# vvvvvw/Sentinel

Measured on AMD Instinct MI355X. Metric: decided entries/sec (whole node) at 1M resources; % of HBM roofline, higher is better.
Workload: dtype int64/f64

## Files before the change

sentinel_amd/csrc/chain.h:

```cpp
#pragma once
#include <hip/hip_runtime.h>
#include <stdint.h>

#include "../../include/sentinel_gpu.h"
#include "dev_types.h"

namespace sg {

__device__ __forceinline__ int64_t j_d2l(double d) {
    if (d != d) return 0;
    if (d >= 9223372036854775807.0) return INT64_MAX;
    if (d <= -9223372036854775808.0) return INT64_MIN;
    return (int64_t)d;
}
__device__ __forceinline__ int32_t j_d2i(double d) {
    if (d != d) return 0;
    if (d >= 2147483647.0) return INT32_MAX;
    if (d <= -2147483648.0) return INT32_MIN;
    return (int32_t)d;
}
__device__ __forceinline__ int32_t j_iadd(int32_t a, int32_t b) { return (int32_t)((uint32_t)a + (uint32_t)b); }
__device__ __forceinline__ int64_t j_round(double a) {
    int64_t bits = __double_as_longlong(a);
    int64_t biased = (bits & 0x7ff0000000000000LL) >> 52;
// ... 89 lines not shown
__device__ __forceinline__ void bkt_add(Bkt& b, int64_t dP, int64_t dB, int64_t dS, int64_t dRT, int64_t dE, int64_t mrt) {
    b.pass += dP; b.block += dB; b.succ += dS; b.rt += dRT; b.exc += dE;
    if (mrt < b.minrt) b.minrt = mrt;
}
__device__ __forceinline__ void bkt_add_if(Bkt& b, bool c, int64_t dP, int64_t dB, int64_t dS, int64_t dRT, int64_t dE,
                                           int64_t mrt) {
    b.pass += c ? dP : 0; b.block += c ? dB : 0; b.succ += c ? dS : 0; b.rt += c ? dRT : 0; b.exc += c ? dE : 0;
    b.minrt = (c && mrt < b.minrt) ? mrt : b.minrt;
}
__device__ __forceinline__ void sec_add(Node& N, int sl, int64_t dP, int64_t dB, int64_t dS, int64_t dRT, int64_t dE,
                                        int64_t mrt) {
    bkt_add_if(N.sb[0], sl == 0, dP, dB, dS, dRT, dE, mrt);
    bkt_add_if(N.sb[1], sl == 1, dP, dB, dS, dRT, dE, mrt);
}
#define SEC_SUM(N, t, f) ((((t) - (N).sb[0].ws <= 1000 && (N).sb[0].ws >= 0) ? (N).sb[0].f : 0) + \
                          (((t) - (N).sb[1].ws <= 1000 && (N).sb[1].ws >= 0) ? (N).sb[1].f : 0))

__device__ __forceinline__ void min_flush(Node& N, Bkt* minb) {
    if (N.mslot >= 0 && (N.mst & MS_DIRTY) && !(N.mst & MS_DETACHED)) minb[N.mslot] = N.mb;
    N.mst &= ~MS_DIRTY;
}
__device__ __forceinline__ void exc_advance(Node& N, const Bkt* minb, int64_t T) {
    if (N.exc_sum_sec >= 0 && T - N.exc_sum_sec >= 60000) {
        N.exc_sum = 0;
    } else if (N.exc_sum_sec < 0) {
        int64_t s = 0;
        for (int k = 0; k < 60; ++k) {
            Bkt b = minb[k];
            if (b.ws >= T - 59000 && b.ws <= T) s += b.exc;
        }
        N.exc_sum = s;
    } else {
        const int64_t x1 = T - 60000;
        for (int64_t x = N.exc_sum_sec - 59000; x <= x1; x += 1000) {
            const int sl = (int)((x / 1000) % 60);
            const Bkt b = sl == N.pfslot ? N.pf : minb[sl];
            if (b.ws == x) N.exc_sum -= b.exc;
        }
    }
    N.exc_sum_sec = T;
}
__device__ __forceinline__ void min_current(Node& N, Bkt* minb, int64_t t, int32_t max_rt, uint32_t pflags) {
    int slot = (int)((t / 1000) % 60);
    int64_t ws = t - t % 1000;
    if (N.mslot == slot && N.mb.ws == ws) return;
    min_flush(N, minb);
    if ((pflags & PF_EXC_COUNT) && N.exc_sum_sec < ws) exc_advance(N, minb, ws);
    Bkt b = slot == N.pfslot ? N.pf : minb[slot];
    N.mslot = slot;
    N.mst = 0;
    if (N.pfslot >= -1) {
        N.pfslot = (slot + 1) % 60;
        N.pf = minb[N.pfslot];
    }
    if (b.ws == ws) { N.mb = b; return; }
    bool back = b.ws > ws;
    bkt_reset(b, ws, max_rt);
    N.mb = b;
    N.mst = back ? MS_DETACHED : MS_DIRTY;
}
__device__ __forceinline__ int64_t min_prev_pass(Node& N, Bkt* minb, int64_t t, int32_t max_rt, uint32_t pflags) {
    min_current(N, minb, t, max_rt, pflags);
    int slot = (int)(((t - 1000) / 1000) % 60);
    Bkt b = minb[slot];
    if (b.ws < 0) return 0;
    if (t - b.ws > 60000) return 0;
    if (b.ws + 1000 < t - 1000) return 0;
// ... 236 lines not shown
```

sentinel_amd/csrc/decide.hip:

```cpp
#include <hip/hip_runtime.h>
#include <stdlib.h>
#include <stdint.h>

#include "authority.h"
#include "chain.h"
#include "aux.h"
#include "pmap.h"

using namespace sg;

#define WAVE 64
#define MAXR 16
#define JMAX_FLOW 4
#define JMAX_DEG 4
#define JMAX_RL 2

__device__ __forceinline__ uint32_t lane_id() { return __lane_id(); }
__device__ __forceinline__ uint64_t lanemask_lt() {
    uint32_t l = lane_id();
    return l == 0 ? 0ull : (~0ull >> (64 - l));
}

#define J8_MAX (1u << 23)
#define SEG_ITEMS 16
// ... 1078 lines not shown
            LPROF(ktc)
        }
        if (r.kind == SG_EV_ENTRY) dec[sg.start + j] = d;
    }
    min_flush(N, C.minb);
    node_store(N, S, res, pg.pflags);
    if (L.mid != NO_ID) pm_store(S, L.mid, L.mp);
    if (L.tid != NO_ID) pm_store(S, L.tid, L.tm);
#pragma unroll
    for (int s = 0; s < NRMAX; ++s) if (s < nr) S.rstate[pg.rule_off + s] = rs[s];
#ifdef SG_KPROF
    if (kp) {
        S.dbg[32] += kta; S.dbg[33] += ktb; S.dbg[34] += ktc; S.dbg[35] += sg.len; S.dbg[36] += 1;
    }
#endif
#undef LPROF
}
template <int NRMAX>
__global__ __launch_bounds__(256) void k_lane(const SEv* __restrict__ recs, const sg_event* __restrict__ ev,
                                              const uint32_t* __restrict__ vals, const Seg* __restrict__ segs,
                                              const uint32_t* __restrict__ order, uint32_t m, DevState S, DevCfg cfg,
                                              int64_t t0, uint32_t* __restrict__ dec, uint32_t* __restrict__ bflags) {
    const uint32_t i = blockIdx.x * blockDim.x + threadIdx.x;
    if (i >= m) return;
    lane_seg<NRMAX>(recs, ev, vals, segs[order[i]], S, cfg, t0, dec, bflags, i);
}

struct MinDelta {
    int32_t p, b, s, rt, e, minrt;
};
struct LiteMin {
    int64_t T;
    MinDelta pd;
    bool fly;
    int64_t fT;
    MinDelta fd;
    Bkt fb;
};
__device__ __forceinline__ void md_zero(MinDelta& d) { d.p = d.b = d.s = d.rt = d.e = 0; d.minrt = INT32_MAX; }
__device__ __forceinline__ bool md_full(const MinDelta& d) { return (uint32_t)(d.p | d.b | d.s | d.rt | d.e) >= 0x40000000u; }
__device__ __forceinline__ Bkt md_apply(Bkt b, int64_t T, const MinDelta& d, int32_t max_rt) {
    if (b.ws > T) return b;
    if (b.ws < T) bkt_reset(b, T, max_rt);
    b.pass += d.p; b.block += d.b; b.succ += d.s; b.rt += d.rt; b.exc += d.e;
    if ((int64_t)d.minrt < b.minrt) b.minrt = d.minrt;
    return b;
}
__device__ __forceinline__ void lm_finish(LiteMin& L, Bkt* minb, int32_t max_rt) {
    if (L.fly) {
        minb[(L.fT / 1000) % 60] = md_apply(L.fb, L.fT, L.fd, max_rt);
        L.fly = false;
    }
}
__device__ __forceinline__ void lm_roll(LiteMin& L, Node& N, Bkt* minb, int64_t T, int32_t max_rt, uint32_t pflags) {
    lm_finish(L, minb, max_rt);
    if (L.T >= 0) {
        L.fb = minb[(L.T / 1000) % 60];
        L.fT = L.T;
        L.fd = L.pd;
        L.fly = true;
    }
    L.T = T;
    md_zero(L.pd);
    if ((pflags & PF_EXC_COUNT) && N.exc_sum_sec < T) {
        if (N.exc_sum_sec < 0) lm_finish(L, minb, max_rt);
        exc_advance(N, minb, T);
    }
}

#ifndef LITE_PL_WAVES
#define LITE_PL_WAVES 1
#endif
template <bool PL>
__global__ __launch_bounds__(256) __attribute__((amdgpu_waves_per_eu(PL ? LITE_PL_WAVES : 2))) void k_lite(const SEv* __restrict__ recs, const sg_event* __restrict__ ev,
                                              const uint32_t* __restrict__ vals, const Seg* __restrict__ segs,
                                              const uint32_t* __restrict__ order, uint32_t m, DevState S, DevCfg cfg,
                                              int64_t t0, uint32_t* __restrict__ dec, uint32_t* __restrict__ bflags) {
    const uint32_t i = blockIdx.x * blockDim.x + threadIdx.x;
    if (i >= m) return;
    const Seg sg = segs[order[i]];
    const uint32_t res = sg.res;
    const Prog pg = S.prog[res];
    if (((pg.xf & XF_PLITE) != 0) != PL) return;
    const int nf = pg.n_flow, nd = pg.n_degrade;
    const DRule* rules = S.rules + pg.rule_off + (PL ? 1 : 0);
    __shared__ DRule spr[PL ? 256 : 1];
    __shared__ PMap smp[PL ? 256 : 1], stm[PL ? 256 : 1];
    DRule& pr = spr[PL ? threadIdx.x : 0];
    PmLaneRef PLM{NO_ID, NO_ID, smp[PL ? threadIdx.x : 0], stm[PL ? threadIdx.x : 0]};
    if (PL) {
        pr = S.rules[pg.rule_off];
        PLM.mid = pr.pmap;
        PLM.mp = S.pmap[pr.pmap];
        PLM.tid = tmap_of(S, pg.tm_base, 0);
        if (PLM.tid != NO_ID) PLM.tm = S.pmap[PLM.tid];
    }
    double fcnt[2] = {0.0, 0.0};
    bool fthr[2] = {false, false};
    uint32_t fslot[2] = {0, 0};
    DegParam dr[2];
    uint32_t dslot[2] = {0, 0};
    RState ds[2];
#pragma unroll
    for (int k = 0; k < 2; ++k) {
        if (k < nf) {
            fcnt[k] = rules[k].count;
            fthr[k] = rules[k].grade == SG_FLOW_GRADE_THREAD;
            fslot[k] = rules[k].slot;
        }
        if (k < nd) {
            dr[k] = deg_param(rules[nf + k]);
            dslot[k] = rules[nf + k].slot;
            ds[k] = S.rstate[pg.rule_off + (PL ? 1 : 0) + nf + k];
        }
    }
#ifdef SG_KPROF
    const bool kp = S.dbg && i == 0;
    unsigned long long kt0 = kp ? __builtin_amdgcn_s_memtime() : 0, kta = 0, ktb = 0, ktc = 0, ktd = 0, ktf = 0, ktg = 0, kth = 0;
#define LPROF(acc)                                                \
    if (kp) {                                                     \
        unsigned long long _n = __builtin_amdgcn_s_memtime();     \
        acc += _n - kt0;                                          \
        kt0 = _n;                                                 \
    }
#else
#define LPROF(acc)
#endif
    Node N;
    node_load(N, S, res);
    const Ctx C{S.minb + (uint64_t)res * 60, cfg.max_rt, pg.pflags};
    LiteMin L;
    L.T = -1;
    L.fly = false;
    md_zero(L.pd);
    const bool has_chain = (N.flags & NI_CHAIN) != 0;
    const bool chain = has_chain && cfg.switch_on;
    if (sg.len && (t0 + recs[sg.start].dt) < (N.sb[0].ws > N.sb[1].ws ? N.sb[0].ws : N.sb[1].ws))
        atomicOr(bflags, BF_BACKWARD);
    uint64_t pm0 = 0, pm1 = 0, pm2 = 0, pm3 = 0;
#ifndef LITE_CH
#define LITE_CH 4
#endif
    constexpr uint32_t CH = LITE_CH;
    const uint4* r4 = reinterpret_cast<const uint4*>(recs + sg.start);
    const uint32_t qmax = sg.len ? sg.len - 1 : 0;
    uint4 cur[CH], nxt[CH];
#pragma unroll
    for (uint32_t k = 0; k < CH; ++k) cur[k] = r4[k < qmax ? k : qmax];
    LPROF(kta)
    for (uint32_t j0 = 0; j0 < sg.len; j0 += CH) {
#pragma unroll
    for (uint32_t k = 0; k < CH; ++k) nxt[k] = r4[j0 + CH + k < qmax ? j0 + CH + k : qmax];
#pragma unroll 1
    for (uint32_t k = 0; k < CH; ++k) {
        const uint4 rw = cur[0];
#pragma unroll
        for (uint32_t m = 0; m + 1 < CH; ++m) cur[m] = cur[m + 1];
        const uint32_t j = j0 + k;
        if (j >= sg.len) break;
        const int32_t rdt = (int32_t)rw.x;
        const uint32_t rx = rw.y;
        const int cntv = (int)(rw.z & 0xFFFFu);
        const int32_t rtv = (int32_t)(rw.z >> 16);
        const uint32_t kind = rw.w & 0xFFu, code = (rw.w >> 16) & 0xFFu;
        const int64_t t = t0 + rdt;
        const int64_t T = t - t % 1000;
        uint32_t d = mk_dec(ST_NOT_ENTRY, 0, 0);
        if (kind == SG_EV_ENTRY) {
            if (!chain) d = mk_dec(ST_NO_CHECK, 0, 0);
            else {
                if (T != L.T || md_full(L.pd)) lm_roll(L, N, C.minb, T, C.max_rt, C.pflags);
                uint32_t status = ST_PASS, slot = 0;
                uint64_t key = NO_KEY;
                if (PL) {
                    N.flags |= NI_PM | ni_tm(0);
                    if ((rw.w >> 8) & SG_F_HAS_ARG)
                        key = S.key_ring[(S.gbase + (vals[sg.start + j] & 0x7FFFFFFFu)) & cfg.ring_mask];
                    if (key != NO_KEY && !param_default_lane(S, pr, PLM.mp, cntv, key, t, bflags)) {
                        status = ST_BLOCK_PARAM;
                        slot = pr.slot;
                    }
                }
#pragma unroll
                for (int k = 0; k < 2; ++k) {
                    if (k < nf && status == ST_PASS) {
                        int32_t cur;
                        if (fthr[k]) cur = N.thread;
                        else { sec_current(N, t, C.max_rt); cur = j_d2i((double)SEC_SUM(N, t, pass)); }
                        if ((double)j_iadd(cur, cntv) > fcnt[k]) { status = ST_BLOCK_FLOW; slot = fslot[k]; }
                    }
                }
                LPROF(ktf)
                const int64_t exc_total = N.exc_sum;
#pragma unroll
                for (int k = 0; k < 2; ++k) {
                    if (k < nd && status == ST_PASS && !degrade_pass(N, C, dr[k], ds[k], t, &exc_total)) {
                        status = ST_BLOCK_DEGRADE;
                        slot = dslot[k];
                    }
                }
                LPROF(ktg)
                const bool passed = status == ST_PASS;
                const int sl = sec_current(N, t, C.max_rt);
                if (passed) {
                    N.thread++;
                    sec_add(N, sl, cntv, 0, 0, 0, 0, INT64_MAX);
                    L.pd.p += cntv;
                } else {
                    sec_add(N, sl, 0, cntv, 0, 0, 0, INT64_MAX);
                    L.pd.b += cntv;
                }
                LPROF(kth)
                if (PL && passed && key != NO_KEY && PLM.tid != NO_ID) thread_add_lane(S, PLM.tm, key, 1, bflags);
                d = passed ? mk_dec(ST_PASS, 0, 0) : mk_dec(status, slot, 0);
                if (passed && j < 256) {
                    const uint64_t b = 1ull << (j & 63);
                    if (j < 64) pm0 |= b; else if (j < 128) pm1 |= b; else if (j < 192) pm2 |= b; else pm3 |= b;
                }
            }
            LPROF(ktb)
        } else {
            bool eff;
            if (code == RC_NONE) eff = kind == SG_EV_EXIT ? chain : has_chain;
            else if (code == RC_PASSED) eff = true;
            else if (code == RC_NOT) eff = false;
            else {
                const uint32_t rel = rx - sg.start;
                if (rel >= j) { atomicOr(bflags, BF_BAD_REF); eff = false; }
                else if (rel < 256) {
                    const uint64_t w = rel < 64 ? pm0 : rel < 128 ? pm1 : rel < 192 ? pm2 : pm3;
                    eff = ((w >> (rel & 63)) & 1) != 0;
                } else eff = st_passed(dec[rx] & 0xFF);
            }
            if (eff && kind == SG_EV_EXIT) {
                if (T != L.T || md_full(L.pd)) lm_roll(L, N, C.minb, T, C.max_rt, C.pflags);
                const int sl = sec_current(N, t, C.max_rt);
                sec_add(N, sl, 0, 0, cntv, rtv, 0, rtv);
                L.pd.s += cntv;
                L.pd.rt += rtv;
                if (rtv < L.pd.minrt) L.pd.minrt = rtv;
                N.thread--;
                const uint32_t rfl = (rw.w >> 8) & 0xFFu;
                if (PL && (rfl & SG_F_EXIT_ARGS) && (N.flags & NI_PM) && (N.flags & ni_tm(0)) && PLM.tid != NO_ID) {
                    uint64_t ref = SG_REF_NONE;
                    if (rfl & RF_OWN_ARGS) ref = S.gbase + (vals[sg.start + j] & 0x7FFFFFFFu);
                    else if (code == RC_BATCH) ref = S.gbase + (vals[rx] & 0x7FFFFFFFu);
                    else if (code == RC_PASSED) ref = ev[vals[sg.start + j] & 0x7FFFFFFFu].aux & SG_REF_NONE;
                    if (ref != SG_REF_NONE) {
                        const uint64_t key = S.key_ring[ref & cfg.ring_mask];
                        if (key != NO_KEY) thread_add_lane(S, PLM.tm, key, -1, bflags);
                    }
                }
            } else if (eff && cntv > 0) {
                if (T != L.T || md_full(L.pd)) lm_roll(L, N, C.minb, T, C.max_rt, C.pflags);
                const int sl = sec_current(N, t, C.max_rt);
                sec_add(N, sl, 0, 0, 0, 0, cntv, INT64_MAX);
                L.pd.e += cntv;
                if (N.exc_sum_sec == T) N.exc_sum += cntv;
            }
            LPROF(ktc)
        }
        if (kind == SG_EV_ENTRY) dec[sg.start + j] = d;
    }
#pragma unroll
    for (uint32_t k = 0; k < CH; ++k) cur[k] = nxt[k];
    }
    lm_finish(L, C.minb, C.max_rt);
    if (L.T >= 0) {
        Bkt* b = C.minb + (L.T / 1000) % 60;
        *b = md_apply(*b, L.T, L.pd, C.max_rt);
    }
    node_store(N, S, res, pg.pflags);
#pragma unroll
    for (int k = 0; k < 2; ++k)
        if (k < nd) S.rstate[pg.rule_off + (PL ? 1 : 0) + nf + k] = ds[k];
    if (PL) {
        pm_store(S, PLM.mid, PLM.mp);
        if (PLM.tid != NO_ID) pm_store(S, PLM.tid, PLM.tm);
    }
    LPROF(ktd)
#ifdef SG_KPROF
    if (kp) {
        S.dbg[32] += kta; S.dbg[33] += ktb; S.dbg[34] += ktc; S.dbg[35] += sg.len; S.dbg[36] += 1; S.dbg[37] += ktd; S.dbg[38] += ktf; S.dbg[39] += ktg; S.dbg[51] += kth;
    }
#endif
#undef LPROF
}

#define DPP_STEP(v, ident, ctrl, rmask, OP) \
    v = OP((uint32_t)__builtin_amdgcn_update_dpp((int)(ident), (int)(v), ctrl, rmask, 0xf, false), v)
#define WAVE_SCAN(v, ident, OP)              \
    do {                                      \
        DPP_STEP(v, ident, 0x111, 0xf, OP);   \
        DPP_STEP(v, ident, 0x112, 0xf, OP);   \
        DPP_STEP(v, ident, 0x114, 0xf, OP);   \
        DPP_STEP(v, ident, 0x118, 0xf, OP);   \
        DPP_STEP(v, ident, 0x142, 0xa, OP);   \
        DPP_STEP(v, ident, 0x143, 0xc, OP);   \
    } while (0)
__device__ __forceinline__ uint32_t op_add(uint32_t a, uint32_t b) { return a + b; }
__device__ __forceinline__ uint32_t op_min(uint32_t a, uint32_t b) { return a < b ? a : b; }
__device__ __forceinline__ uint32_t op_max(uint32_t a, uint32_t b) { return a > b ? a : b; }
__device__ __forceinline__ void wave_total64(uint32_t v, uint64_t* dst) {
    uint32_t lo = v & 0xFFFFu, hi = v >> 16;
// ... 2346 lines not shown
```

sentinel_amd/csrc/dev_types.h:

```cpp
#pragma once
#include <hip/hip_runtime.h>
#include <stdint.h>

#include "../../include/sentinel_gpu.h"

namespace sg {

struct AuthDesc;

struct Bkt {
    int64_t ws;
    int64_t pass;
    int64_t block;
    int64_t exc;
    int64_t succ;
    int64_t rt;
    int64_t occ;
    int64_t minrt;
};
static_assert(sizeof(Bkt) == 64, "Bkt must be 64 B");

#define NO_KEY 0xFFFFFFFFFFFFFFFFull

enum : uint32_t {
// ... 114 lines not shown
    int64_t stamp[PM_BKT];
};
static_assert(sizeof(PBucket) == 128, "PBucket must be one 128-byte line");
struct PData {
    int64_t v0;
    int32_t v1;
    uint32_t pad;
};
static_assert(sizeof(PData) == 16, "PData must be 16 B");
#define PM_MIN_NB 2u
enum { PC_NEXT = 0, PC_FLOOR = 1, PC_RESCUES = 2, PC_RESCUE = 3, PC_WORDS = 4 };
__host__ __device__ inline uint32_t map_buckets(uint32_t cap) { return (2u * cap + PM_BKT - 1) / PM_BKT > 2u ? (2u * cap + PM_BKT - 1) / PM_BKT : 2u; }
struct PMap {
    uint64_t base;
    uint64_t bm;
    int64_t clock;
    int64_t thr;
    uint32_t nb;
    uint32_t cap;
    uint32_t live;
    uint32_t rb_log2;
    uint32_t pad[4];
};
static_assert(sizeof(PMap) == 64, "PMap must be 64 B");
#define PM_BASE_CAP 4000u
#define PM_TOTAL_CAP 200000u
#define PQ_MAX_CAP 8176u

enum : uint8_t { ST_PASS = 0, ST_PASS_WAIT = 1, ST_BLOCK_FLOW = 2, ST_BLOCK_DEGRADE = 3, ST_BLOCK_PARAM = 4,
                 ST_NO_CHECK = 5, ST_BLOCK_UPSTREAM = 6, ST_BLOCK_AUTHORITY = 7, ST_NOT_ENTRY = 0xFF };

#define HEAD_OFF 16384u
#define TABLES_ALL 32768u
struct DevCfg {
    int32_t max_rt;
    int32_t occupy_timeout;
    int32_t max_chain;
    int32_t switch_on;
    uint64_t reserved0;
    uint64_t ring_mask;
    uint32_t dbg_flags;
    uint32_t heads;
};

struct Seg {
    uint32_t res;
    uint32_t start;
    uint32_t len;
    uint32_t bin;
};
#define SEG_AUXP 0x80u
#define SEG_PV 0x40u
#define SEG_PVT 0x100u

struct PvSeg {
    uint32_t ok;
    uint32_t n;
    uint32_t off;
    uint32_t mid;
    uint32_t rk;
    uint32_t ch0;
    uint32_t nch;
    uint32_t fbits;
    uint32_t freach;
    int32_t peak;
    uint32_t tm0;
    uint32_t sub;
};

struct PvBuf {
    uint64_t* key;
    uint32_t* pos;
// ... 135 lines not shown
    unsigned long long* dbg;
    uint32_t* sink;
    const Link* link;
    const uint32_t* bst;
    uint32_t* pend;
    Span* spans;
    uint32_t* nspan;
    uint32_t span_cap;
    uint32_t epoch;
    uint32_t skip_ok;
    uint32_t skip_min;
    const sg_event_ext* ext;
    const sg_arg* args;
    AuxNode* aux_tab;
    uint32_t* aux_count;
    uint32_t aux_cap;
    uint32_t max_ctx;
    uint64_t aux_mask;
    const AuthDesc* auth;
    const uint32_t* auth_ids;
};

enum : uint32_t { BF_PRIORITIZED = 1,
                  BF_PQ_INVARIANT = 2,
                  BF_PTAB_FULL = 4,
                  BF_BAD_RES = 8, BF_BAD_REF = 16,
                  BF_BACKWARD = 32, BF_TSPAN = 64,
                  BF_BAD_ARGS = 512,
                  BF_AUX_FULL = 1024,
                  BF_POOL_FULL = 2048,
                  BF_MULTI_LINK = 128,
                  BF_ZERO_CNT = 256,
                  BF_TINY_FALLBACK = 4096,
                  BF_TINY_REJECTED = 8192 };

struct SEv {
    int32_t dt;
    uint32_t x;
    uint16_t cnt;
    uint16_t rt;
    uint8_t kind;
    uint8_t flags;
    uint8_t code;
    uint8_t pad;
};
static_assert(sizeof(SEv) == 16, "SEv must be 16 B");
enum : uint8_t {
    RC_NONE = 0,
    RC_BATCH = 1,
    RC_PASSED = 2,
    RC_NOT = 3,
    RC_PREV = 4
};

enum : uint32_t {
    BIN_J16 = 0,
    BIN_J4 = 1,
    BIN_J1 = 2,
    BIN_PQ16 = 3,
    BIN_PQ4 = 4,
    BIN_J8 = 5,
    BIN_LANE = 6,
    LANE_BINS = 19,
    BIN_LANE16 = BIN_LANE + LANE_BINS,
    BIN_LITE = BIN_LANE16 + LANE_BINS,
    N_BINS = BIN_LITE + LANE_BINS
};
// ... 3 lines not shown
```

sentinel_amd/csrc/engine.cpp:

```cpp
#include <hip/hip_runtime.h>

#include <algorithm>
#include <array>
#include <cmath>
#include <cstdint>
#include <cstdio>
#include <cstdlib>
#include <cstring>
#include <functional>
#include <map>
#include <set>
#include <string>
#include <unordered_map>
#include <vector>

#include "../../include/sentinel_gpu.h"
#include "authority.h"
#include "dev_types.h"
#include "pmap.h"

namespace sg {
hipError_t launch_rs_first(const sg_event* ev, uint64_t n, uint32_t max_res, uint64_t gbase, const uint8_t* ring,
                           uint64_t ring_mask, int32_t max_rt, SEv* rec_o, uint32_t* keys, uint32_t* vals,
                           uint32_t* ghist, uint32_t nblocks, uint32_t* bflags, int64_t* t0_out, uint32_t* prio,
// ... 473 lines not shown

    std::unordered_map<std::string, uint32_t> ids;
    std::vector<std::string> names;
    uint32_t n_chains = 0;

    bool flow_loaded = false, deg_loaded = false, par_loaded = false;
    std::vector<std::string> last_flow, last_deg, last_par;
    std::vector<FlowR> flows;
    std::vector<DegR> degs;
    std::vector<ParamR> params;
    std::vector<std::vector<int>> res_flow, res_deg, res_par;
    std::map<std::string, uint32_t> psid_of;
    uint32_t next_psid = 1;
    std::map<uint32_t, uint32_t> rmap_cap;
    std::set<uint64_t> tmaps;
    std::vector<uint64_t> pmap_key;
    std::unordered_map<uint32_t, uint32_t> pmap_index;
    std::vector<uint32_t> tm_base;
    uint64_t n_pslot = 0;
    uint64_t pool_nb = 0;
    unsigned long long* d_pool_next = nullptr;
    uint4* d_pmoves = nullptr;
    PBucket* d_pbkt2 = nullptr;
    PData* d_pdat2 = nullptr;
    uint32_t* d_pcwork = nullptr;
    uint64_t pmoves_cap = 0;
    unsigned long long* h_pool_next = nullptr;
    uint64_t n_compact = 0;
    uint64_t pool2_nb = 0;
    uint32_t n_dev_rules = 0;

    Bkt* d_sec = nullptr;
    Bkt* d_minb = nullptr;
    NodeInfo* d_info = nullptr;
    Prog* d_prog = nullptr;
    DRule* d_rules = nullptr;
    RState* d_rstate = nullptr;
    DHot* d_hot = nullptr;
    PMap* d_pmap = nullptr;
    PBucket* d_pbkt = nullptr;
    PData* d_pdat = nullptr;
    uint64_t* d_pbm = nullptr;
    uint32_t* d_ppre = nullptr;
    uint32_t* d_tmid = nullptr;
    uint8_t* d_ring = nullptr;
    uint32_t rules_cap = 0, hot_cap = 0;

    struct BatchSlot {
        sg_event* d_ev = nullptr;
        uint32_t* d_out = nullptr;
        uint32_t *d_k0 = nullptr, *d_v0 = nullptr, *d_k1 = nullptr, *d_v1 = nullptr;
        uint32_t *d_hist = nullptr, *d_part = nullptr, *d_flag = nullptr, *d_pos = nullptr, *d_order = nullptr;
        uint32_t *d_posof = nullptr, *d_dec = nullptr, *d_blkcnt = nullptr, *d_prev = nullptr;
        SEv *d_recs = nullptr, *d_rec_o = nullptr;
        uint32_t* d_ccnt = nullptr;
        bool radix = false;
        uint32_t nhot = 0;
        Seg* d_segs = nullptr;
        uint64_t* d_cand = nullptr;
        uint32_t* d_bsmall = nullptr;
        sg_event_ext* d_ext = nullptr;
        sg_arg* d_args = nullptr;
        uint64_t ext_cap = 0, args_cap = 0;
        uint32_t* d_ashort = nullptr;
        uint64_t *d_apiece = nullptr, *d_amulti = nullptr, *d_along = nullptr;
        uint64_t aux_cap_n = 0;
// ... 210 lines not shown
        HIPCHK(hipMalloc(&B.d_pend, c * 4));
        HIPCHK(hipMalloc(&B.d_spans, (c / SPAN_CHUNK + 65536) * sizeof(Span)));
    }
    e->span_cap = (uint32_t)(c / SPAN_CHUNK + 65536);
    e->cap_n = c;
    activate(e, e->cur);
    return SG_OK;
}

static int collect(sg_engine* e, int k) {
    auto& B = e->slot[k];
    if (!B.pending) return SG_OK;
    B.pending = false;
    HIPCHK(hipEventSynchronize(B.ev[4]));
    float g = 0, d = 0, p = 0;
    (void)hipEventElapsedTime(&g, B.ev[0], B.ev[1]);
    (void)hipEventElapsedTime(&d, B.ev[2], B.ev[3]);
    (void)hipEventElapsedTime(&p, B.ev[3], B.ev[4]);
    (void)hipGetLastError();
    e->last_ms[0] = g; e->last_ms[1] = d; e->last_ms[2] = p; e->last_ms[3] = (double)g + d + p;
    e->tlog.push_back({(double)g, (double)d, (double)p, (double)g + d + p});
    if (e->tlog.size() > 4096) e->tlog.erase(e->tlog.begin(), e->tlog.begin() + 2048);
    uint32_t bflags = 0;
    HIPCHK(hipMemcpyAsync(&bflags, B.d_bsmall, 4, hipMemcpyDeviceToHost, e->gstream));
    uint32_t nspan = 0;
    HIPCHK(hipMemcpyAsync(&nspan, B.d_bsmall + 120, 4, hipMemcpyDeviceToHost, e->gstream));
    HIPCHK(hipStreamSynchronize(e->gstream));
    e->spans_total += nspan;
    if (bflags & BF_BAD_REF)
        return fail(SG_EINVAL, "an EXIT/TRACE references an event that is not an earlier ENTRY of the same resource");
    if (bflags & BF_BACKWARD)
        return fail(SG_EINVAL, "event timestamps must be non-decreasing across batches (SURVEY Q3)");
    if (bflags & BF_AUX_FULL) return fail(SG_ECAPACITY, "origin/context node pool full (raise aux_node_capacity)");
    if (bflags & BF_PQ_INVARIANT)
        e->fatal = "internal error: a k_pq tile's presorted key subset did not match its accesses";
    else if (bflags & BF_POOL_FULL)
        e->fatal = "the hot-parameter map pool is used up (raise param_table_log2)";
    else if (bflags & BF_PTAB_FULL)
        e->fatal = "a hot-parameter map table could not place a key (its map holds a ghost entry)";
    if (bflags & (BF_PQ_INVARIANT | BF_PTAB_FULL | BF_POOL_FULL)) return fail(SG_ECAPACITY, e->fatal + " -- engine unusable");
    return SG_OK;
}
static inline const AuthDesc* dev_auth(const sg_engine* e) { return e->auth_on ? e->d_auth : nullptr; }
static inline const uint32_t* dev_auth_ids(const sg_engine* e) { return e->auth_on ? e->d_auth_ids : nullptr; }

static int drain(sg_engine* e) {
    int rc = SG_OK;
    for (int i = 0; i < 2; ++i) {
        int r = collect(e, (e->cur + i) & 1);
        if (r && !rc) rc = r;
    }
    HIPCHK(hipStreamSynchronize(e->stream));
    return rc;
}


static uint32_t rule_map_cap(int64_t duration_sec) {
    const int64_t c = (int64_t)PM_BASE_CAP * std::max<int64_t>(duration_sec, 1);
    return (uint32_t)std::min<int64_t>(c, PM_TOTAL_CAP);
}

int upload_rules(sg_engine* e, bool reset_flow_state, bool reset_deg_state, bool reset_par_state) {
    uint32_t R = e->cfg.max_resources;
    std::vector<Prog> prog(R);
    std::vector<DRule> rules;
    std::vector<RState> rst;
// ... 392 lines not shown
        e->cfg.aux_node_capacity = (uint32_t)cap;
        if (hipMalloc(&e->d_auxtab, slots * sizeof(AuxNode)) != hipSuccess || hipMalloc(&e->d_auxcnt, 4) != hipSuccess ||
            hipMemsetAsync(e->d_auxtab, 0xFF, slots * sizeof(AuxNode), e->stream) != hipSuccess ||
            hipMemsetAsync(e->d_auxcnt, 0, 4, e->stream) != hipSuccess)
            return bad(fail(SG_ENOMEM, "device allocation of the origin/context node table failed"));
    }
    if (hipMemsetAsync(e->d_prog, 0, R * sizeof(Prog), e->stream) != hipSuccess ||
        hipMemsetAsync(e->d_ring, 0xFF, 1ull << cfg.status_ring_log2, e->stream) != hipSuccess ||
        hipMemsetAsync(e->d_prio, 0, R * 4, e->stream) != hipSuccess ||
        hipMemsetAsync(e->d_hot_tab, 0xFF, R * 2, e->stream) != hipSuccess ||
        launch_init_state(e->d_sec, e->d_minb, e->d_info, e->d_borrow, (uint32_t)R, e->stream) != hipSuccess ||
        hipStreamSynchronize(e->stream) != hipSuccess)
        return bad(fail(SG_EDEVICE, "device initialisation failed"));
    for (auto& s : e->bin_stream)
        if (hipStreamCreateWithPriority(&s, hipStreamNonBlocking, prio_hi) != hipSuccess) return bad(fail(SG_EDEVICE, "stream"));
    if (hipEventCreateWithFlags(&e->fork, hipEventDisableTiming) != hipSuccess ||
        hipEventCreateWithFlags(&e->fork0, hipEventDisableTiming) != hipSuccess ||
        hipEventCreateWithFlags(&e->grown, hipEventDisableTiming) != hipSuccess)
        return bad(fail(SG_EDEVICE, "event"));
    for (auto& v : e->join)
        if (hipEventCreateWithFlags(&v, hipEventDisableTiming) != hipSuccess) return bad(fail(SG_EDEVICE, "event"));
    if (const char* d = std::getenv("SG_DEBUG")) {
        if (d[0] == '1' && hipMalloc(&e->d_dbg, 64 * 8) == hipSuccess) (void)hipMemset(e->d_dbg, 0, 64 * 8);
    }
    if (const char* f = std::getenv("SG_DEBUG_FLAGS")) e->dbg_flags = (uint32_t)std::strtoul(f, nullptr, 0);
    e->radix_group = (e->dbg_flags & 8192) != 0;
    if (const char* f = std::getenv("SG_PROF_BIN")) e->prof_bin = std::atoi(f);
    if (const char* v = std::getenv("SG_LANE_MAX")) { e->lane_max = (uint32_t)std::strtoul(v, nullptr, 0); e->bins_pinned = true; }
    if (const char* v = std::getenv("SG_J1_MAX")) { e->j1_max = (uint32_t)std::strtoul(v, nullptr, 0); e->bins_pinned = true; }
    if (const char* v = std::getenv("SG_HEAD_MIN")) e->head_min = (uint32_t)std::strtoul(v, nullptr, 0);
    if (const char* v = std::getenv("SG_J4_MAX")) { e->j4_max = (uint32_t)std::strtoul(v, nullptr, 0); e->bins_pinned = true; }
    if (const char* v = std::getenv("SG_PIPELINE")) e->pipeline = v[0] == '1';
    if (const char* v = std::getenv("SG_TINY")) e->tiny_on = v[0] != '0';
    if (const char* v = std::getenv("SG_RADIX_BELOW")) e->radix_below = std::strtoull(v, nullptr, 0);
    if (const char* v = std::getenv("SG_TOK_WIDE")) e->tok_wide = std::atoi(v) == 512 ? 512u : 1024u;
    if (const char* v = std::getenv("SG_TOK_LIGHT")) e->tok_light = (uint32_t)std::strtoul(v, nullptr, 0);
    if (const char* v = std::getenv("SG_TOK_NS")) e->tok_ns = v[0] == '1';
    e->ns_names.push_back("default");
    e->ns_of["default"] = 0;
    e->ns_limit.push_back((double)cfg.cluster_max_allowed_qps);
    e->ns_conn.push_back(0);
    if (const char* v = std::getenv("SG_J1_STREAM")) e->j1_stream = std::atoi(v);
    if (const char* v = std::getenv("SG_PQ")) e->pq_on = v[0] != '0';
    if (const char* v = std::getenv("SG_MIX")) e->mix_on = v[0] != '0';
    if (const char* v = std::getenv("SG_MIX_PQ")) e->mix_pq = v[0] != '0';
    if (const char* v = std::getenv("SG_PV_PQ")) e->pv_pq = v[0] != '0';
    if (const char* v = std::getenv("SG_PV")) e->pv_on = v[0] != '0';
    e->pvt_on = e->pv_on;
    if (const char* v = std::getenv("SG_PVT")) e->pvt_on = v[0] != '0';
    if (const char* v = std::getenv("SG_PQ_WIDE")) e->pq_wide = (uint32_t)std::strtoul(v, nullptr, 0);
    if (const char* v = std::getenv("SG_SKIP_MIN")) {
        e->skip_min = std::max<uint32_t>(1u, (uint32_t)std::strtoul(v, nullptr, 0));
        e->skip_pinned = true;
    }
    *out = e;
    return SG_OK;
}

extern "C" int sgx_timing_log(sg_engine* e, double* out, int cap) {
    if (!e || !out) return 0;
    (void)drain(e);
    int k = 0;
    for (; k < cap && k < (int)e->tlog.size(); ++k)
        for (int j = 0; j < 4; ++j) out[4 * k + j] = e->tlog[k][j];
    e->tlog.clear();
    return k;
// ... 1047 lines not shown
    }
    const uint32_t hot_min = (uint32_t)std::max<uint64_t>(64, n / 8192);
    if (!B.radix)
        HIPCHK(launch_hot_build(e->d_segs, e->d_bsmall + 1, mb, hot_min, R, e->d_hot_tab, e->d_hot_list, e->nhot,
                                e->d_bsmall + 76, gs));
    uint32_t head[77];
    static_assert(8 + N_BINS + 1 <= 72, "head layout");
    HIPCHK(hipMemcpyAsync(head, e->d_bsmall, sizeof(head), hipMemcpyDeviceToHost, gs));
    HIPCHK(hipEventRecord(B.ev[1], gs));
    HIPCHK(hipStreamSynchronize(gs));
    if (!B.radix) e->nhot = std::min<uint32_t>(head[76], hot_max());
    const uint32_t m = head[1];
    const uint32_t nprev = head[3];
    int64_t t0 = 0;
    std::memcpy(&t0, head + 4, 8);
    uint32_t bflags = head[0];
    if (bflags & BF_BAD_RES) return fail(SG_EINVAL, "event res_id >= max_resources");
    if (bflags & BF_BAD_REF)
        return fail(SG_EINVAL, "an EXIT/TRACE references an event that is not an earlier ENTRY of the same resource");
    if (bflags & BF_TSPAN) return fail(SG_EINVAL, "a batch must span less than 2^31 ms");
    if (bflags & BF_BACKWARD) return fail(SG_EINVAL, "event timestamps must be non-decreasing (SURVEY Q3)");
    if (bflags & BF_BAD_ARGS)
        return fail(SG_EINVAL, "an sg_event_ext names args outside the table (or more than SG_MAX_ARGS, or a bad kind)");
    const uint32_t* off = head + 8;
    uint32_t bin_n[N_BINS];
    for (int b = 0; b < N_BINS; ++b) bin_n[b] = off[b + 1] - off[b];
    DevCfg dc;
    std::memset(&dc, 0, sizeof(dc));
    dc.max_rt = e->cfg.statistic_max_rt;
    dc.occupy_timeout = e->cfg.occupy_timeout_ms;
    dc.max_chain = e->cfg.max_slot_chain_size;
    dc.switch_on = e->cfg.switch_on;
    dc.ring_mask = ring_mask;
    dc.dbg_flags = e->dbg_flags;
    dc.heads = e->has_head ? 1u : 0u;
    DevState S{};
    std::memset(&S, 0, sizeof(S));
    S.sec = e->d_sec;
    S.minb = e->d_minb;
    S.info = e->d_info;
    S.prog = e->d_prog;
    S.rules = e->d_rules;
    S.rstate = e->d_rstate;
    S.hot = e->d_hot;
    S.pmap = e->d_pmap;
    S.pbkt = e->d_pbkt;
    S.pdat = e->d_pdat;
    S.pbm = e->d_pbm;
    S.ppre = e->d_ppre;
    S.tmid = e->d_tmid;
    S.ring = e->d_ring;
    S.sink = e->d_sink;
    S.borrow = e->d_borrow;
    S.prio = e->d_prio;
    S.key_ring = e->d_keyring;
    S.gbase = e->gbase;
    S.link = e->d_link;
    S.bst = e->d_bst;
    S.pend = e->d_pend;
    S.spans = e->d_spans;
    S.nspan = e->d_bsmall + 120;
    S.span_cap = e->span_cap;
    S.epoch = e->epoch;
    S.skip_ok = !(bflags & (BF_MULTI_LINK | BF_ZERO_CNT)) && !(e->dbg_flags & 4) ? 1u : 0u;
    S.skip_min = (!e->skip_pinned && n < SHARD_BATCH) ? std::min<uint32_t>(e->skip_min, 8192) : e->skip_min;
    S.ext = dev_ext;
// ... 223 lines not shown
    if (!is_device_ptr(ev)) {
        HIPCHK(hipMemcpyAsync(e->d_ev, ev, n * sizeof(sg_event), hipMemcpyHostToDevice, st));
        dev_ev = e->d_ev;
    }
    uint32_t* dev_out = host_out ? e->d_out : out;
    const sg_event_ext* dev_ext = ext;
    const sg_arg* dev_args = n_args ? args : nullptr;
    if (ext && !is_device_ptr(ext)) {
        if (n > B.ext_cap) {
            dfree(B.d_ext);
            B.ext_cap = std::max<uint64_t>(n, 1u << 16);
            HIPCHK(hipMalloc(&B.d_ext, B.ext_cap * sizeof(sg_event_ext)));
        }
        HIPCHK(hipMemcpyAsync(B.d_ext, ext, n * sizeof(sg_event_ext), hipMemcpyHostToDevice, st));
        dev_ext = B.d_ext;
    }
    if (n_args && !is_device_ptr(args)) {
        if (n_args > B.args_cap) {
            dfree(B.d_args);
            B.args_cap = std::max<uint64_t>(n_args, 1u << 16);
            HIPCHK(hipMalloc(&B.d_args, B.args_cap * sizeof(sg_arg)));
        }
        HIPCHK(hipMemcpyAsync(B.d_args, args, n_args * sizeof(sg_arg), hipMemcpyHostToDevice, st));
        dev_args = B.d_args;
    }
    if (++e->epoch == 0) e->epoch = 1;
    DevCfg dc;
    std::memset(&dc, 0, sizeof(dc));
    dc.max_rt = e->cfg.statistic_max_rt;
    dc.occupy_timeout = e->cfg.occupy_timeout_ms;
    dc.max_chain = e->cfg.max_slot_chain_size;
    dc.switch_on = e->cfg.switch_on;
    dc.ring_mask = (1ull << e->cfg.status_ring_log2) - 1;
    dc.dbg_flags = e->dbg_flags;
    dc.heads = e->has_head ? 1u : 0u;
    DevState S{};
    std::memset(&S, 0, sizeof(S));
    S.sec = e->d_sec; S.minb = e->d_minb; S.info = e->d_info; S.prog = e->d_prog; S.rules = e->d_rules;
    S.rstate = e->d_rstate; S.hot = e->d_hot; S.pmap = e->d_pmap; S.pbkt = e->d_pbkt; S.pdat = e->d_pdat;
    S.pbm = e->d_pbm; S.ppre = e->d_ppre; S.tmid = e->d_tmid; S.ring = e->d_ring; S.sink = e->d_sink;
    S.borrow = e->d_borrow; S.prio = e->d_prio; S.key_ring = e->d_keyring; S.gbase = e->gbase; S.link = e->d_link;
    S.bst = e->d_bst; S.pend = e->d_pend; S.spans = e->d_spans; S.nspan = e->d_bsmall + 120; S.span_cap = e->span_cap;
    S.epoch = e->epoch; S.skip_ok = 0; S.skip_min = e->skip_min; S.ext = dev_ext; S.args = dev_args;
    S.aux_tab = e->d_auxtab; S.aux_count = e->d_auxcnt; S.aux_cap = e->cfg.aux_node_capacity; S.aux_mask = e->aux_mask;
    S.max_ctx = SG_MAX_CONTEXTS;
    S.auth = dev_auth(e);
    S.auth_ids = dev_auth_ids(e);
    const int cap = e->cfg.max_slot_chain_size;
    const uint32_t grants = cap <= 0 ? 1u : e->n_chains >= (uint32_t)cap ? 2u : 0u;
    HIPCHK(launch_tiny(dev_ev, (uint32_t)n, S, dc, e->cfg.max_resources, e->d_prio, e->d_comp, n_args, grants,
                       e->d_pool_next, e->pool_nb, e->epoch, e->d_recs, e->d_v0, e->d_dec, e->d_segs, e->d_bsmall,
                       dev_out, st));
    uint32_t bflags = 0;
    HIPCHK(hipMemcpyAsync(&bflags, e->d_bsmall, 4, hipMemcpyDeviceToHost, st));
    if (host_out) HIPCHK(hipMemcpyAsync(out, dev_out, n * 4, hipMemcpyDeviceToHost, st));
    if (e->pool_nb) HIPCHK(hipMemcpyAsync(e->h_pool_next, e->d_pool_next, PC_WORDS * 8, hipMemcpyDeviceToHost, st));
    HIPCHK(hipStreamSynchronize(st));
    if (bflags & BF_TINY_FALLBACK) return TINY_FALLBACK;
    if (bflags & BF_TINY_REJECTED) {
        if (bflags & BF_BAD_RES) return fail(SG_EINVAL, "event res_id >= max_resources");
        if (bflags & BF_BAD_REF)
            return fail(SG_EINVAL, "an EXIT/TRACE references an event that is not an earlier ENTRY of the same resource");
        if (bflags & BF_TSPAN) return fail(SG_EINVAL, "a batch must span less than 2^31 ms");
        if (bflags & BF_BACKWARD) return fail(SG_EINVAL, "event timestamps must be non-decreasing (SURVEY Q3)");
        return fail(SG_EINVAL, "an sg_event_ext names args outside the table (or more than SG_MAX_ARGS, or a bad kind)");
    }
// ... 163 lines not shown
        ex(sec[1], out->second[1]);
        for (int i = 0; i < 60; ++i) ex(mb[i], out->minute[i]);
        for (int i = 0; i < 2; ++i)
            if (bor[2 * i] >= 0) {
                out->borrow[i].window_start = bor[2 * i];
                out->borrow[i].pass = bor[2 * i + 1];
                out->borrow[i].min_rt = e->cfg.statistic_max_rt;
            }
    } else {
        for (int i = 0; i < 60; ++i) out->minute[i].window_start = -1;
    }
    out->cur_thread_num = chain ? ni.thread : 0;
    out->has_chain = chain ? 1 : 0;
    return SG_OK;
}

int sg_snapshot_metrics(sg_engine* e, int64_t now_ms, sg_metric_node* out, uint64_t cap, uint64_t* n) {
    if (!e || !n) return fail(SG_EINVAL, "null argument");
    HIPCHK(hipSetDevice(e->device));
    if (int rc = drain(e)) return rc;
    uint32_t R = (uint32_t)std::min<size_t>(e->names.size(), e->cfg.max_resources);
    if (R == 0) { *n = 0; return SG_OK; }
    if (!e->d_snap_cnt) {
        HIPCHK(hipMalloc(&e->d_snap_cnt, (uint64_t)e->cfg.max_resources * 4));
        HIPCHK(hipMalloc(&e->d_snap_off, (uint64_t)e->cfg.max_resources * 4));
    }
    const bool dev_out = out && is_device_ptr(out);
    if (!dev_out && cap > e->snap_cap) {
        dfree(e->d_snap_out);
        HIPCHK(hipMalloc(&e->d_snap_out, std::max<uint64_t>(cap, 1) * sizeof(sg_metric_node)));
        e->snap_cap = cap;
    }
    if (!e->d_part) { int rc = ensure_batch(e, 1); if (rc) return rc; }
    HIPCHK(launch_snapshot(e->d_minb, e->d_info, R, now_ms, e->cfg.statistic_max_rt, e->d_snap_cnt, e->d_snap_off,
                           e->d_part, e->d_small + 3, dev_out ? out : e->d_snap_out, dev_out || out ? cap : 0,
                           e->stream));
    uint32_t total = 0;
    HIPCHK(hipMemcpyAsync(&total, e->d_small + 3, 4, hipMemcpyDeviceToHost, e->stream));
    HIPCHK(hipStreamSynchronize(e->stream));
    uint64_t k = std::min<uint64_t>(total, cap);
    if (k && out && !dev_out)
        HIPCHK(hipMemcpy(out, e->d_snap_out, k * sizeof(sg_metric_node), hipMemcpyDeviceToHost));
    *n = total;
    return SG_OK;
}

int sg_cluster_set_connected_count(sg_engine* e, int64_t flow_id, int32_t connected) {
    if (!e) return fail(SG_EINVAL, "null engine");
    if (int rc = drain(e)) return rc;
    auto it = e->cmap.find(flow_id);
    auto pt = e->pmap.find(flow_id);
    if (it == e->cmap.end() && pt == e->pmap.end()) return fail(SG_ENOTFOUND, "no cluster rule with this flowId");
    if (it != e->cmap.end()) {
        e->cflows[it->second].connected = connected;
        HIPCHK(hipMemcpy(&e->d_cflow[it->second].connected, &connected, sizeof(int32_t), hipMemcpyHostToDevice));
    }
    if (pt != e->pmap.end()) {
        e->pflows[pt->second].connected = connected;
        HIPCHK(hipMemcpy(&e->d_pflow[pt->second].connected, &connected, sizeof(int32_t), hipMemcpyHostToDevice));
    }
    return SG_OK;
}

static int ensure_ns(sg_engine* e) {
    if (e->d_nslim) return SG_OK;
    std::vector<NsLimiter> z(SG_MAX_NAMESPACES);
// ... 301 lines not shown
```

Baseline: 4.153 billion.

## Skip stale minute-bucket loads in k_lite and batch decision stores

In the lite kernel, the deferred in-flight minute-bucket read-modify-write is replaced by a high-water mark. When a bucket's second is newer than anything previously stored (node second buckets or the snapshot high mark), it is written fresh without being loaded first. Decision words are now held in a small register shift window and flushed per chunk, the node and record loads are hoisted ahead of the early return, and rule loads become branch-free clamped reads. The exception-sum scan also stops once the sum reaches zero. These changes aim to cut global loads and scattered stores per event, at the cost of relying on a new staleness invariant (checked only under an opt-in debug flag) and more register pressure.

```diff
diff --git a/sentinel_amd/csrc/chain.h b/sentinel_amd/csrc/chain.h
--- a/sentinel_amd/csrc/chain.h
+++ b/sentinel_amd/csrc/chain.h
@@ -145,7 +145,7 @@
         N.exc_sum = s;
     } else {
         const int64_t x1 = T - 60000;
-        for (int64_t x = N.exc_sum_sec - 59000; x <= x1; x += 1000) {
+        for (int64_t x = N.exc_sum_sec - 59000; x <= x1 && N.exc_sum != 0; x += 1000) {
             const int sl = (int)((x / 1000) % 60);
             const Bkt b = sl == N.pfslot ? N.pf : minb[sl];
             if (b.ws == x) N.exc_sum -= b.exc;
diff --git a/sentinel_amd/csrc/decide.hip b/sentinel_amd/csrc/decide.hip
--- a/sentinel_amd/csrc/decide.hip
+++ b/sentinel_amd/csrc/decide.hip
@@ -1134,10 +1134,7 @@
 struct LiteMin {
     int64_t T;
     MinDelta pd;
-    bool fly;
-    int64_t fT;
-    MinDelta fd;
-    Bkt fb;
+    int64_t H;
 };
 __device__ __forceinline__ void md_zero(MinDelta& d) { d.p = d.b = d.s = d.rt = d.e = 0; d.minrt = INT32_MAX; }
 __device__ __forceinline__ bool md_full(const MinDelta& d) { return (uint32_t)(d.p | d.b | d.s | d.rt | d.e) >= 0x40000000u; }
@@ -1148,26 +1145,35 @@
     if ((int64_t)d.minrt < b.minrt) b.minrt = d.minrt;
     return b;
 }
-__device__ __forceinline__ void lm_finish(LiteMin& L, Bkt* minb, int32_t max_rt) {
-    if (L.fly) {
-        minb[(L.fT / 1000) % 60] = md_apply(L.fb, L.fT, L.fd, max_rt);
-        L.fly = false;
-    }
-}
-__device__ __forceinline__ void lm_roll(LiteMin& L, Node& N, Bkt* minb, int64_t T, int32_t max_rt, uint32_t pflags) {
-    lm_finish(L, minb, max_rt);
-    if (L.T >= 0) {
-        L.fb = minb[(L.T / 1000) % 60];
-        L.fT = L.T;
-        L.fd = L.pd;
-        L.fly = true;
-    }
+__device__ __forceinline__ void lm_put(LiteMin& L, Bkt* minb, int32_t max_rt, bool check, uint32_t* bflags) {
+    if (L.T < 0) return;
+    Bkt* p = minb + (L.T / 1000) % 60;
+    if (L.T > L.H) {
+        if (check && p->ws >= L.T) atomicOr(bflags, BF_LITE_STALE);
+        Bkt b;
+        bkt_reset(b, L.T, max_rt);
+        b.pass = L.pd.p; b.block = L.pd.b; b.succ = L.pd.s; b.rt = L.pd.rt; b.exc = L.pd.e;
+        if ((int64_t)L.pd.minrt < b.minrt) b.minrt = L.pd.minrt;
+        *p = b;
+        L.H = L.T;
+    } else {
+        *p = md_apply(*p, L.T, L.pd, max_rt);
+    }
+}
+__device__ __forceinline__ void lm_roll(LiteMin& L, Node& N, Bkt* minb, int64_t T, int32_t max_rt, uint32_t pflags,
+                                        bool check, uint32_t* bflags) {
+    lm_put(L, minb, max_rt, check, bflags);
     L.T = T;
     md_zero(L.pd);
-    if ((pflags & PF_EXC_COUNT) && N.exc_sum_sec < T) {
-        if (N.exc_sum_sec < 0) lm_finish(L, minb, max_rt);
-        exc_advance(N, minb, T);
-    }
+    if ((pflags & PF_EXC_COUNT) && N.exc_sum_sec < T) exc_advance(N, minb, T);
+}
+template <uint32_t CH>
+__device__ __forceinline__ void lite_flush(uint32_t* __restrict__ dec, uint32_t base, uint32_t n, const uint32_t (&w)[CH],
+                                           uint32_t& mask) {
+#pragma unroll
+    for (uint32_t m = 0; m < CH; ++m)
+        if ((mask >> m) & 1u) dec[base + m - (CH - n)] = w[m];
+    mask = 0;
 }
 
 #ifndef LITE_PL_WAVES
@@ -1183,6 +1189,17 @@
     const Seg sg = segs[order[i]];
     const uint32_t res = sg.res;
     const Prog pg = S.prog[res];
+    Node N;
+    node_load(N, S, res);
+#ifndef LITE_CH
+#define LITE_CH 4
+#endif
+    constexpr uint32_t CH = LITE_CH;
+    const uint4* r4 = reinterpret_cast<const uint4*>(recs + sg.start);
+    const uint32_t qmax = sg.len ? sg.len - 1 : 0;
+    uint4 cur[CH], nxt[CH];
+#pragma unroll
+    for (uint32_t k = 0; k < CH; ++k) cur[k] = r4[k < qmax ? k : qmax];
     if (((pg.xf & XF_PLITE) != 0) != PL) return;
     const int nf = pg.n_flow, nd = pg.n_degrade;
     const DRule* rules = S.rules + pg.rule_off + (PL ? 1 : 0);
@@ -1203,17 +1220,17 @@
     DegParam dr[2];
     uint32_t dslot[2] = {0, 0};
     RState ds[2];
-#pragma unroll
-    for (int k = 0; k < 2; ++k) {
-        if (k < nf) {
-            fcnt[k] = rules[k].count;
-            fthr[k] = rules[k].grade == SG_FLOW_GRADE_THREAD;
-            fslot[k] = rules[k].slot;
-        }
-        if (k < nd) {
-            dr[k] = deg_param(rules[nf + k]);
-            dslot[k] = rules[nf + k].slot;
-            ds[k] = S.rstate[pg.rule_off + (PL ? 1 : 0) + nf + k];
+    if (nf + nd) {
+        const int last = nf + nd - 1;
+#pragma unroll
+        for (int k = 0; k < 2; ++k) {
+            const int fi = k < last ? k : last, di = nf + k < last ? nf + k : last;
+            fcnt[k] = rules[fi].count;
+            fthr[k] = rules[fi].grade == SG_FLOW_GRADE_THREAD;
+            fslot[k] = rules[fi].slot;
+            dr[k] = deg_param(rules[di]);
+            dslot[k] = rules[di].slot;
+            ds[k] = S.rstate[pg.rule_off + (PL ? 1 : 0) + di];
         }
     }
 #ifdef SG_KPROF
@@ -1228,29 +1245,30 @@
 #else
 #define LPROF(acc)
 #endif
-    Node N;
-    node_load(N, S, res);
     const Ctx C{S.minb + (uint64_t)res * 60, cfg.max_rt, pg.pflags};
     LiteMin L;
     L.T = -1;
-    L.fly = false;
     md_zero(L.pd);
+    {
+        const int64_t sw = N.sb[0].ws > N.sb[1].ws ? N.sb[0].ws : N.sb[1].ws;
+        const int64_t sh = sw < 0 ? -1 : sw - sw % 1000;
+        L.H = sh > cfg.snap_hi ? sh : cfg.snap_hi;
+    }
+    const bool lchk = (cfg.dbg_flags & LITE_CHECK) != 0;
     const bool has_chain = (N.flags & NI_CHAIN) != 0;
     const bool chain = has_chain && cfg.switch_on;
     if (sg.len && (t0 + recs[sg.start].dt) < (N.sb[0].ws > N.sb[1].ws ? N.sb[0].ws : N.sb[1].ws))
         atomicOr(bflags, BF_BACKWARD);
     uint64_t pm0 = 0, pm1 = 0, pm2 = 0, pm3 = 0;
-#ifndef LITE_CH
-#define LITE_CH 4
+#ifndef LITE_HOLD
+#define LITE_HOLD 1
 #endif
-    constexpr uint32_t CH = LITE_CH;
-    const uint4* r4 = reinterpret_cast<const uint4*>(recs + sg.start);
-    const uint32_t qmax = sg.len ? sg.len - 1 : 0;
-    uint4 cur[CH], nxt[CH];
-#pragma unroll
-    for (uint32_t k = 0; k < CH; ++k) cur[k] = r4[k < qmax ? k : qmax];
+    uint32_t dw[CH], dmask = 0;
+#pragma unroll
+    for (uint32_t k = 0; k < CH; ++k) dw[k] = 0;
     LPROF(kta)
     for (uint32_t j0 = 0; j0 < sg.len; j0 += CH) {
+    if (j0) lite_flush<CH>(dec, sg.start + j0 - CH, CH, dw, dmask);
 #pragma unroll
     for (uint32_t k = 0; k < CH; ++k) nxt[k] = r4[j0 + CH + k < qmax ? j0 + CH + k : qmax];
 #pragma unroll 1
@@ -1271,7 +1289,7 @@
         if (kind == SG_EV_ENTRY) {
             if (!chain) d = mk_dec(ST_NO_CHECK, 0, 0);
             else {
-                if (T != L.T || md_full(L.pd)) lm_roll(L, N, C.minb, T, C.max_rt, C.pflags);
+                if (T != L.T || md_full(L.pd)) lm_roll(L, N, C.minb, T, C.max_rt, C.pflags, lchk, bflags);
                 uint32_t status = ST_PASS, slot = 0;
                 uint64_t key = NO_KEY;
                 if (PL) {
@@ -1332,10 +1350,13 @@
                 else if (rel < 256) {
                     const uint64_t w = rel < 64 ? pm0 : rel < 128 ? pm1 : rel < 192 ? pm2 : pm3;
                     eff = ((w >> (rel & 63)) & 1) != 0;
-                } else eff = st_passed(dec[rx] & 0xFF);
+                } else {
+                    if (rel >= j0) lite_flush<CH>(dec, sg.start + j0, k, dw, dmask);
+                    eff = st_passed(dec[rx] & 0xFF);
+                }
             }
             if (eff && kind == SG_EV_EXIT) {
-                if (T != L.T || md_full(L.pd)) lm_roll(L, N, C.minb, T, C.max_rt, C.pflags);
+                if (T != L.T || md_full(L.pd)) lm_roll(L, N, C.minb, T, C.max_rt, C.pflags, lchk, bflags);
                 const int sl = sec_current(N, t, C.max_rt);
                 sec_add(N, sl, 0, 0, cntv, rtv, 0, rtv);
                 L.pd.s += cntv;
@@ -1354,7 +1375,7 @@
                     }
                 }
             } else if (eff && cntv > 0) {
-                if (T != L.T || md_full(L.pd)) lm_roll(L, N, C.minb, T, C.max_rt, C.pflags);
+                if (T != L.T || md_full(L.pd)) lm_roll(L, N, C.minb, T, C.max_rt, C.pflags, lchk, bflags);
                 const int sl = sec_current(N, t, C.max_rt);
                 sec_add(N, sl, 0, 0, 0, 0, cntv, INT64_MAX);
                 L.pd.e += cntv;
@@ -1362,16 +1383,23 @@
             }
             LPROF(ktc)
         }
+#if LITE_HOLD
+#pragma unroll
+        for (uint32_t m = 0; m + 1 < CH; ++m) dw[m] = dw[m + 1];
+        dw[CH - 1] = d;
+        dmask = (dmask >> 1) | (kind == SG_EV_ENTRY ? 1u << (CH - 1) : 0u);
+#else
         if (kind == SG_EV_ENTRY) dec[sg.start + j] = d;
+#endif
     }
 #pragma unroll
     for (uint32_t k = 0; k < CH; ++k) cur[k] = nxt[k];
     }
-    lm_finish(L, C.minb, C.max_rt);
-    if (L.T >= 0) {
-        Bkt* b = C.minb + (L.T / 1000) % 60;
-        *b = md_apply(*b, L.T, L.pd, C.max_rt);
-    }
+    if (sg.len) {
+        const uint32_t jl = (sg.len - 1) / CH * CH;
+        lite_flush<CH>(dec, sg.start + jl, sg.len - jl, dw, dmask);
+    }
+    lm_put(L, C.minb, C.max_rt, lchk, bflags);
     node_store(N, S, res, pg.pflags);
 #pragma unroll
     for (int k = 0; k < 2; ++k)
diff --git a/sentinel_amd/csrc/dev_types.h b/sentinel_amd/csrc/dev_types.h
--- a/sentinel_amd/csrc/dev_types.h
+++ b/sentinel_amd/csrc/dev_types.h
@@ -170,12 +170,13 @@
 
 #define HEAD_OFF 16384u
 #define TABLES_ALL 32768u
+#define LITE_CHECK 65536u
 struct DevCfg {
     int32_t max_rt;
     int32_t occupy_timeout;
     int32_t max_chain;
     int32_t switch_on;
-    uint64_t reserved0;
+    int64_t snap_hi;
     uint64_t ring_mask;
     uint32_t dbg_flags;
     uint32_t heads;
@@ -377,7 +378,8 @@
                   BF_MULTI_LINK = 128,
                   BF_ZERO_CNT = 256,
                   BF_TINY_FALLBACK = 4096,
-                  BF_TINY_REJECTED = 8192 };
+                  BF_TINY_REJECTED = 8192,
+                  BF_LITE_STALE = 16384 };
 
 struct SEv {
     int32_t dt;
diff --git a/sentinel_amd/csrc/engine.cpp b/sentinel_amd/csrc/engine.cpp
--- a/sentinel_amd/csrc/engine.cpp
+++ b/sentinel_amd/csrc/engine.cpp
@@ -529,6 +529,7 @@
 
     Bkt* d_sec = nullptr;
     Bkt* d_minb = nullptr;
+    int64_t snap_hi = -1;
     NodeInfo* d_info = nullptr;
     Prog* d_prog = nullptr;
     DRule* d_rules = nullptr;
@@ -805,6 +806,8 @@
     if (bflags & BF_BACKWARD)
         return fail(SG_EINVAL, "event timestamps must be non-decreasing across batches (SURVEY Q3)");
     if (bflags & BF_AUX_FULL) return fail(SG_ECAPACITY, "origin/context node pool full (raise aux_node_capacity)");
+    if (bflags & BF_LITE_STALE)
+        return fail(SG_ESTATE, "internal error (SG_LITE_CHECK): k_lite stored a minute bucket without a load that was not stale");
     if (bflags & BF_PQ_INVARIANT)
         e->fatal = "internal error: a k_pq tile's presorted key subset did not match its accesses";
     else if (bflags & BF_POOL_FULL)
@@ -1263,6 +1266,7 @@
     if (const char* v = std::getenv("SG_J4_MAX")) { e->j4_max = (uint32_t)std::strtoul(v, nullptr, 0); e->bins_pinned = true; }
     if (const char* v = std::getenv("SG_PIPELINE")) e->pipeline = v[0] == '1';
     if (const char* v = std::getenv("SG_TINY")) e->tiny_on = v[0] != '0';
+    if (const char* v = std::getenv("SG_LITE_CHECK")) { if (v[0] == '1') e->dbg_flags |= LITE_CHECK; }
     if (const char* v = std::getenv("SG_RADIX_BELOW")) e->radix_below = std::strtoull(v, nullptr, 0);
     if (const char* v = std::getenv("SG_TOK_WIDE")) e->tok_wide = std::atoi(v) == 512 ? 512u : 1024u;
     if (const char* v = std::getenv("SG_TOK_LIGHT")) e->tok_light = (uint32_t)std::strtoul(v, nullptr, 0);
@@ -2376,6 +2380,7 @@
     dc.max_chain = e->cfg.max_slot_chain_size;
     dc.switch_on = e->cfg.switch_on;
     dc.ring_mask = ring_mask;
+    dc.snap_hi = e->snap_hi;
     dc.dbg_flags = e->dbg_flags;
     dc.heads = e->has_head ? 1u : 0u;
     DevState S{};
@@ -2665,6 +2670,7 @@
     dc.max_chain = e->cfg.max_slot_chain_size;
     dc.switch_on = e->cfg.switch_on;
     dc.ring_mask = (1ull << e->cfg.status_ring_log2) - 1;
+    dc.snap_hi = e->snap_hi;
     dc.dbg_flags = e->dbg_flags;
     dc.heads = e->has_head ? 1u : 0u;
     DevState S{};
@@ -2894,6 +2900,7 @@
         e->snap_cap = cap;
     }
     if (!e->d_part) { int rc = ensure_batch(e, 1); if (rc) return rc; }
+    e->snap_hi = std::max(e->snap_hi, now_ms - now_ms % 1000);
     HIPCHK(launch_snapshot(e->d_minb, e->d_info, R, now_ms, e->cfg.statistic_max_rt, e->d_snap_cnt, e->d_snap_off,
                            e->d_part, e->d_small + 3, dev_out ? out : e->d_snap_out, dev_out || out ? cap : 0,
                            e->stream));
```

Measured after the change: 4.331 billion (median of 6 runs). 4.3% higher.
